# vvvwo/KSS-ICP

Hardware: AMD Instinct MI355X
Metric: icp_iterations_per_sec (higher is better)
Workload: dtype f32; 1 GPU; C2: one 100000x100000 uniform-sphere pair per GPU, 50 fixed ICP iterations + fitness pass per step (exact NN + cov reduce + host 3x3 SVD), R_z(10deg), jitter 1e-3; n_src=100000, n_tgt=100000, pairs_per_gpu=1, nn_engine=cell list + brute-force fallback, nn_arithmetic=reference (no fma)

## Files before the change

### kss-icp_amd/csrc/kss_api.hip

```cpp
#pragma clang fp contract(off)

#include "kss_ctx.hpp"

extern "C" {

int kss_version(void) { return KSS_VERSION; }

const char* kss_status_string(int s) {
    switch (s) {
        case KSS_OK: return "ok";
        case KSS_ERR_ARG: return "invalid argument";
        case KSS_ERR_HIP: return "HIP runtime error";
        case KSS_ERR_NOMEM: return "out of memory";
        case KSS_ERR_NODEVICE: return "no usable GPU device";
        case KSS_ERR_CAPACITY: return "output buffer too small";
        case KSS_ERR_RCCL: return "RCCL error";
        case KSS_ERR_DEGENERATE: return "degenerate point-to-plane system";
        default: return "unknown status";
    }
}

const char* kss_last_error(const kss_ctx* ctx) { return ctx ? ctx->err.c_str() : ""; }

static int ctx_create_common(int device_id, void* stream, bool borrow, kss_ctx** out) {
// ... 63 lines not shown

void* kss_ctx_stream(kss_ctx* c) { return c ? (void*)c->stream : nullptr; }

int kss_ctx_set_nn_mode(kss_ctx* c, int nn_mode) {
    if (!c || nn_mode < KSS_NN_AUTO || nn_mode > KSS_NN_GRID) return KSS_ERR_ARG;
    c->nn_mode = nn_mode;
    return KSS_OK;
}

int kss_profile_enable(kss_ctx* c, int on) {
    if (!c) return KSS_ERR_ARG;
    c->prof = on > 0 ? on : 0;
    for (int k = 0; k < KSS_K_COUNT; ++k) c->prof_tick[k] = 0;
    if (c->prof) {
        HIPCHK(c, hipSetDevice(c->device));
        while (c->ev_pool.size() < 4096) {
            kss_ctx::EvPair ep;
            if (hipEventCreate(&ep.a) != hipSuccess) break;
            if (hipEventCreate(&ep.b) != hipSuccess) { hipEventDestroy(ep.a); break; }
            c->ev_pool.push_back(ep);
        }
    }
    return KSS_OK;
}
int kss_grid_stats(kss_ctx* c, double out[8]) {
    if (!c || !out) return KSS_ERR_ARG;
    for (int k = 0; k < 8; ++k) out[k] = c->grid_stats[k];
    return KSS_OK;
}
int kss_debug_grid_evals(kss_ctx* c, double out[2]) {
    if (!c || !out) return KSS_ERR_ARG;
    out[0] = c->evals_sum; out[1] = c->evals_launches;
    c->evals_sum = 0.0; c->evals_launches = 0.0;
    return KSS_OK;
}

int kss_debug_grid_stamps(kss_ctx* c, unsigned long long* out, int64_t cap) {
    if (!c || !out) return KSS_ERR_ARG;
    if (c->stamps_nblk > 0 && c->g_stamps.p) {
        hipStreamSynchronize(c->stream);
        c->last_stamps.resize((size_t)c->stamps_nblk * 16);
        if (hipMemcpy(c->last_stamps.data(), (const unsigned long long*)c->g_stamps.p + (size_t)(c->stamps_seq & 1) * c->stamps_nblk * 16,
                      c->last_stamps.size() * sizeof(unsigned long long), hipMemcpyDeviceToHost) != hipSuccess) return KSS_ERR_HIP;
    }
    const int64_t n = std::min<int64_t>(cap, (int64_t)c->last_stamps.size());
    for (int64_t i = 0; i < n; ++i) out[i] = c->last_stamps[(size_t)i];
    return (int)n;
}
int kss_profile_reset(kss_ctx* c) {
    if (!c) return KSS_ERR_ARG;
    HIPCHK(c, hipStreamSynchronize(c->stream));
    prof_collect(c);
    for (int k = 0; k < KSS_K_COUNT; ++k) { c->prof_ms[k] = 0; c->prof_n[k] = 0; }
    return KSS_OK;
}
int kss_profile_event_overhead(kss_ctx* c, double* ms) {
    if (!c || !ms) return KSS_ERR_ARG;
    HIPCHK(c, hipSetDevice(c->device));
    hipEvent_t a = nullptr, b = nullptr;
    HIPCHK(c, hipEventCreate(&a));
    HIPCHK(c, hipEventCreate(&b));
    for (int i = 0; i < 16; ++i) launch_empty(c->stream);
    HIPCHK(c, hipStreamSynchronize(c->stream));
    double tot = 0.0;
    const int reps = 200;
    for (int i = 0; i < reps; ++i) {
// ... 977 lines not shown
```

### kss-icp_amd/csrc/kss_ctx.hpp

```cpp
#pragma once
#include <dlfcn.h>
#include <hip/hip_runtime.h>

#include <algorithm>
#include <atomic>
#include <chrono>
#include <cmath>
#include <cstdio>
#include <cstdlib>
#include <cstring>
#include <mutex>
#include <string>
#include <thread>
#include <vector>

#include "kss_internal.hpp"
#include "kss_host_pool.hpp"

using namespace kss;

struct DevBuf {
    void* p = nullptr;
    size_t cap = 0;
};

struct kss_ctx {
    int device = 0;
    int cu_count = 0;
    hipStream_t stream = nullptr;
    bool own_stream = false;
    std::string err;
    int nn_mode = KSS_NN_AUTO;
    double grid_stats[8] = {0, 0, 0, 0, 0, 0, 0, 0};
    double last_setup_ms = 0, last_loop_ms = 0;
    double t_launch_us = 0, t_wait_us = 0, t_host_us = 0;
    bool timing = false;
    bool tables_staged = false;
    int64_t stats_ns = -1, stats_nt = -1;

    DevBuf tgt4, src0, cur[2], keys, partials, sums, nn_work, red_work, pair_red, state, cs, scratch_a,
        scratch_b, scratch_c, stage_src, stage_tgt, stage_idx, stage_d2, stage_out, g_counts, g_start, g_cursor,
        g_bsums, g_sorted, g_list, g_count, g_bbox, g_partials, g_start2, g_pairs, g_stamps, g_pos, g_nnst, res_pos, res_wc, res_perm, pack_seg, reg_s, reg_t, reg_p, reg_all, reg_f, reg_g, oct_pts, oct_cen, oct_a, oct_b, oct_tmp, pre_partials, pre_state, g_rowpair, g_gate;
    DevBuf p2l_idx, p2l_d2, p2l_perm, p2l_rows, p2l_nrm, p2l_n64;
    DevBuf trim_rows, trim_state;
    HostPool pool;
    std::vector<kss_ctx*> workers;
    std::vector<unsigned long long> last_stamps;
    int stamps_nblk = 0; unsigned long long stamps_seq = 0;
    std::vector<float> h_bbox;
    unsigned int* h_box = nullptr; unsigned int* h_box_dev = nullptr; size_t h_box_bytes = 0;
    unsigned box_tag = 0; int box_rows = 0;
    double evals_sum = 0.0, evals_launches = 0.0;
    void* h_sums = nullptr;  size_t h_sums_cap = 0;
    void* h_sums_dev = nullptr;
    void* h_p2l = nullptr; size_t h_p2l_cap = 0;
    void* h_p2l_dev = nullptr;
    unsigned long long* h_seq = nullptr;
    unsigned long long* h_seq_dev = nullptr;
    size_t h_seq_bytes = 0;
    struct Gated {
        int supported = -1;
        bool want_next = false;
        bool pending = false;
        bool chain = false;
        int steps_left = 0;
        int max_steps = 1;
        int slot = 0;
        unsigned long long seq = 0;
        int32_t stamp = 0;
        const void* d_in = nullptr; void* d_out = nullptr;
        bool fma = false, full = false, want_full = false; double max_d2 = 0.0;
    } gated;
    bool ws_dirty = false;
    bool defer_wait = false;
    PairState* h_xf = nullptr; PairState* h_xf_dev = nullptr;
    bool fit_last = false;
    bool nn_have = false;
    PairState* bar_state = nullptr; int bar_state_cap = 0; bool bar_state_failed = false;
    unsigned int* gate_bar = nullptr;
    unsigned int* res_gate = nullptr; int res_gate_cap = 0; bool res_gate_failed = false;
    unsigned res_launches = 0;
    double res_passes = 0.0;
    int cand_cap = 0, cand_cap_pad = -1, cand_cap_fma = -1;
    int spec_judge = -1; double spec_threshold = 0.0; bool spec_ran = false, spec_cancelled = false;
    std::chrono::steady_clock::time_point res_backoff[2] = {};
    unsigned long long seq = 0;
    void* h_state = nullptr; size_t h_state_cap = 0;

    int prof = 0;
    unsigned prof_tick[KSS_K_COUNT] = {};
    struct EvPair { hipEvent_t a, b; };
    std::vector<EvPair> ev[KSS_K_COUNT];
    std::vector<EvPair> ev_pool;
    double prof_ms[KSS_K_COUNT] = {0};
    int64_t prof_n[KSS_K_COUNT] = {0};
};

// ... 126 lines not shown
```

### kss-icp_amd/csrc/kss_engine.hip

```cpp
#pragma clang fp contract(off)

#include <emmintrin.h>

#include "kss_ctx.hpp"

namespace kss {

static int restore_zero_at_rest(kss_ctx* c);
static bool resident_gate_available(kss_ctx* c, int npairs);

static int resident_rows_limit(kss_ctx* c) {
    if (c->cu_count <= 0) {
        hipDeviceProp_t prop;
        c->cu_count = hipGetDeviceProperties(&prop, c->device) == hipSuccess && prop.multiProcessorCount > 0 ? prop.multiProcessorCount : 1;
        (void)hipGetLastError();
    }
    return c->cu_count;
}

constexpr int PUB_PAIRS = 32;
static int ensure_pub(kss_ctx* c, int npairs = PUB_PAIRS);

struct PairGeom {
    int64_t ns, nt;
// ... 547 lines not shown
    }
    return c->gated.supported == 1;
}

static void gated_release(kss_ctx* c, const PairState& st, int skip) {
    if (c->gate_bar) {
        int words[16];
        std::memcpy(words, &st, sizeof st);
        words[14] = skip;
        unsigned int* slot = c->gate_bar + 32 * c->gated.slot;
        static const long torn_at = getenv("KSS_TEST_TORN_GATE") ? atol(getenv("KSS_TEST_TORN_GATE")) : -1;
        static long released = 0;
        const bool torn = ++released == torn_at;
        for (int pass = torn ? 0 : 1; pass < 2; ++pass) {
            for (int g = 0; g < 5; ++g) {
                const unsigned tag = (unsigned)c->gated.stamp + kss_mix3((unsigned)words[3 * g], (unsigned)words[3 * g + 1], (unsigned)words[3 * g + 2]);
                const int w1 = pass == 0 && g == 1 ? words[3 * g + 1] ^ 0x00010000 : words[3 * g + 1];
                const __m128i v = _mm_set_epi32((int)tag, words[3 * g + 2], w1, words[3 * g]);
                _mm_store_si128((__m128i*)(slot + 4 * g), v);
            }
            _mm_sfence();
            if (pass == 0) {
                const auto t0 = std::chrono::steady_clock::now();
                while (std::chrono::duration<double, std::micro>(std::chrono::steady_clock::now() - t0).count() < 200.0) __builtin_ia32_pause();
            }
        }
    } else {
        PairState* rec = &c->h_xf[c->gated.slot];
        for (int k = 0; k < 12; ++k) rec->m[k] = st.m[k];
        rec->active = st.active; rec->apply = st.apply; rec->pad[0] = skip;
        __atomic_store_n(&rec->pad[1], c->gated.stamp, __ATOMIC_RELEASE);
    }
    kss_ctx::Gated& G = c->gated;
    if (!skip && --G.steps_left > 0) {
        G.slot ^= 1;
        G.stamp += 1;
        G.seq += 1;
        const void* in = G.d_out; G.d_out = const_cast<void*>(G.d_in); G.d_in = in;
    } else {
        G.pending = false;
        G.steps_left = 0;
    }
}

static void gated_cancel(kss_ctx* c) {
    if (!c->gated.pending) return;
    PairState none;
    std::memset(&none, 0, sizeof none);
    gated_release(c, none, 1);
}

struct GatedGuard {
    kss_ctx* c;
    explicit GatedGuard(kss_ctx* c_) : c(c_) {}
    ~GatedGuard() { gated_cancel(c); c->gated.want_next = false; }
};

static PassArgs pass_args(kss_ctx* c, const IcpPlan& pl, const float4* d_in, float4* d_out, double max_d2,
                          int32_t* d_idx_out, float* d_d2_out) {
    PassArgs a;
    std::memset(&a, 0, sizeof a);
    a.src_in = d_in; a.src_out = d_out;
    a.cell_start = (const int32_t*)c->g_start.p + 1;
    a.sorted = (const float4*)c->g_sorted.p;
    a.tgt4 = (const float4*)c->tgt4.p;
    a.nn_win = (float4*)c->g_pos.p;
    a.nn_state = (float2*)c->g_nnst.p;
    static const float skin = getenv("KSS_SKIN") ? (float)atof(getenv("KSS_SKIN")) : 0.25f;
    a.skin = skin;
    a.chain_len = 1;
    static const int gate_polls = getenv("KSS_GATE_POLLS") ? atoi(getenv("KSS_GATE_POLLS")) : (1 << 22);
    a.gate_polls = gate_polls;
    a.chained = d_in != (const float4*)c->src0.p ? 1 : c->fit_last ? 2 : 0;
    a.src_last0 = (const float4*)c->cur[0].p; a.src_last1 = (const float4*)c->cur[1].p;
    a.keys = (unsigned long long*)c->keys.p;
    a.list = (int32_t*)c->g_list.p; a.list_count = (int32_t*)c->g_count.p;
    a.total_rows = pl.total_rows;
    static const bool noprev = getenv("KSS_GRID_NOPREV") != nullptr;
    a.use_prev = !noprev && c->nn_have ? 1 : 0;
    a.max_d2 = max_d2;
    a.rows = (Granule*)c->partials.p;
    a.pub = c->h_seq_dev;
    a.idx_out = d_idx_out; a.d2_out = d_d2_out;
    {
        static const long torn_at = getenv("KSS_TEST_TORN_SLOT") ? atol(getenv("KSS_TEST_TORN_SLOT")) : -1;
        static long launches = 0;
        a.test_torn = torn_at > 0 && ++launches == torn_at ? 1 : 0;
    }
    if (pl.gridb) {
        a.pairs = (const GridPairDev*)c->g_pairs.p;
        a.row_pair = (const int32_t*)c->g_rowpair.p;
        a.defer_pairs = pl.npairs > resident_rows_limit(c) ? pl.npairs : 0;
    } else {
        a.pair0 = pl.gpairs[0];
    }
    return a;
}

static int nn_pass(kss_ctx* c, const IcpPlan& pl, bool fma, const float4* d_in, float4* d_out, double max_d2,
            int32_t* d_idx_out, float* d_d2_out, bool full, const int* active = nullptr) {
    PairState* hs = (PairState*)c->h_state;
    if (pl.grid) {
        PassArgs a = pass_args(c, pl, d_in, d_out, max_d2, d_idx_out, d_d2_out);
        const int nblk = grid_pass_blocks(pl.total_rows);
        static const int stamps_mode = getenv("KSS_GRID_STAMPS") ? atoi(getenv("KSS_GRID_STAMPS")) : 0;
        unsigned long long* stamps2 = nullptr;
        if (stamps_mode == 1) {
            KCHK(ensure(c, c->g_stamps, (size_t)nblk * 16 * sizeof(unsigned long long)));
            HIPCHK(c, hipMemsetAsync(c->g_stamps.p, 0, (size_t)nblk * 16 * sizeof(unsigned long long), c->stream));
            a.stamps = (unsigned long long*)c->g_stamps.p;
        } else if (stamps_mode == 2) {
            KCHK(ensure(c, c->g_stamps, (size_t)nblk * 32 * sizeof(unsigned long long)));
            stamps2 = (unsigned long long*)c->g_stamps.p;
            c->stamps_nblk = nblk;
        }
        const auto tl0 = c->timing ? std::chrono::steady_clock::now() : std::chrono::steady_clock::time_point();
        unsigned long long want_seq = 0;
        bool via_gate = false;
        kss_ctx::Gated& G = c->gated;
        const bool plain_args = !a.stamps && !d_idx_out && !d_d2_out;
        if (G.pending && G.d_in == (const void*)d_in && G.d_out == (void*)d_out && G.fma == fma && G.full == full && G.max_d2 == max_d2 && plain_args) {
            want_seq = G.seq;
            c->seq = std::max(c->seq, G.seq);
            if (G.chain && c->prof > 0) c->prof_n[KSS_K_GRID_CHAIN_PASS] += 1;
            via_gate = true;
            static const long drop_at = getenv("KSS_TEST_DROP_GATE") ? atol(getenv("KSS_TEST_DROP_GATE")) : -1;
            static long releases = 0;
            if (++releases == drop_at) { G.pending = false; G.steps_left = 0; }
            else gated_release(c, hs[0], 0);
        } else {
            gated_cancel(c);
            ProfScope ps(c, KSS_K_GRID_NN);
            a.ps0 = hs[0];
            a.seq = ++c->seq;
            if (stamps2) a.stamps = stamps2 + (size_t)(a.seq & 1) * nblk * 16;
            launch_grid_pass(c->stream, fma, full, false, true, a);
            c->nn_have = true;
            want_seq = c->seq;
        }
        HIPCHK(c, hipGetLastError());
        const bool next_sampled = c->prof == 1 || (c->prof > 1 && c->prof_tick[KSS_K_GRID_NN] % (unsigned)c->prof == 0);
        static const bool want_chain = getenv("KSS_CHAIN") == nullptr || atoi(getenv("KSS_CHAIN")) != 0;
        int len = 1;
        if (G.want_next && !G.pending && plain_args && gated_available(c) && want_chain && c->gate_bar &&
            (pl.total_rows <= resident_rows_limit(c) || pl.total_rows == 1))
            len = std::max(1, std::min(G.max_steps, 1 << 16));
        if (G.want_next && !G.pending && plain_args && gated_available(c) && (len > 1 || !next_sampled)) {
            if (c->prof > 1 && len == 1) ++c->prof_tick[KSS_K_GRID_NN];
            float4* nxt_out = d_out == (float4*)c->cur[0].p ? (float4*)c->cur[1].p : (float4*)c->cur[0].p;
            G.slot ^= 1;
            G.stamp = (G.stamp + 1) & 0x7fffffff;
            if (G.stamp == 0 || G.stamp > 0x7fffffff - len - 1) G.stamp = 1;
            PassArgs n = pass_args(c, pl, d_out, nxt_out, max_d2, nullptr, nullptr);
            n.ps0 = hs[0];
            n.gate_seq = G.stamp;
            if (c->gate_bar) {
                n.state = nullptr;
                n.gate_dev = c->gate_bar;
                n.gate_slot = G.slot;
                n.chain_len = len;
                n.src_alt = d_out;
            } else {
                n.state = c->h_xf_dev + G.slot;
                n.gate_dev = (unsigned int*)c->g_gate.p;
            }
            n.seq = c->seq + 1;
            if (stamps2) n.stamps = stamps2 + (size_t)(n.seq & 1) * nblk * 16;
            if (len > 1) {
                ProfScope ps(c, KSS_K_GRID_CHAIN, true);
                launch_grid_pass(c->stream, fma, G.want_full, false, true, n);
            } else {
                launch_grid_pass(c->stream, fma, G.want_full, false, true, n);
            }
            G.chain = len > 1;
            G.pending = true; G.steps_left = len; G.seq = n.seq; G.d_in = d_out; G.d_out = nxt_out; G.fma = fma; G.full = G.want_full; G.max_d2 = max_d2;
            if (hipGetLastError() != hipSuccess) { gated_cancel(c); G.supported = 0; }
        }
        const auto tl1 = c->timing ? std::chrono::steady_clock::now() : std::chrono::steady_clock::time_point();
        {
            bool not_published = false;
            int rcw = wait_seq(c, 1, want_seq, nullptr, &not_published);
            if (rcw != KSS_OK && via_gate && not_published) {
                G.pending = false; G.steps_left = 0;
                c->err.clear();
                std::fprintf(stderr, "[kss] a waiting kernel was not answered in time and left; the pass is launched again\n");
                c->ws_dirty = true;
                KCHK(restore_zero_at_rest(c));
                ProfScope ps(c, KSS_K_GRID_NN);
                a.ps0 = hs[0];
                a.seq = ++c->seq;
                launch_grid_pass(c->stream, fma, full, false, true, a);
                HIPCHK(c, hipGetLastError());
                want_seq = c->seq;
                rcw = wait_seq(c, 1, want_seq);
            }
            KCHK(rcw);
        }
        if (stamps2) c->stamps_seq = want_seq;
        if (c->timing) {
            const auto tl2 = std::chrono::steady_clock::now();
            c->t_launch_us += std::chrono::duration<double, std::micro>(tl1 - tl0).count();
            c->t_wait_us += std::chrono::duration<double, std::micro>(tl2 - tl1).count();
        }
        if (a.stamps && !stamps2) {
            c->last_stamps.resize((size_t)nblk * 16);
            HIPCHK(c, hipMemcpy(c->last_stamps.data(), a.stamps, c->last_stamps.size() * sizeof(unsigned long long), hipMemcpyDeviceToHost));
            for (int b = 0; b < nblk; ++b) c->evals_sum += (double)c->last_stamps[(size_t)b * 16 + 10];
            c->evals_launches += 1.0;
        }
        if (((const double*)c->h_sums)[NSUMS - 1] > 0.0) {
            gated_cancel(c);
            c->gated.want_next = false;
            KCHK(stage_tables(c, pl));
            {
                PairState one;
                std::memset(&one, 0, sizeof one);
                one.active = 1;
                HIPCHK(c, hipMemcpy(c->state.p, &one, sizeof one, hipMemcpyHostToDevice));
            }
            if (getenv("KSS_LIST_CHECK")) {
                HIPCHK(c, hipStreamSynchronize(c->stream));
                int32_t cnt = -1;
                HIPCHK(c, hipMemcpy(&cnt, c->g_count.p, sizeof cnt, hipMemcpyDeviceToHost));
                const int64_t ns0 = pl.g[0].ns;
                std::vector<int32_t> l((size_t)std::max<int64_t>(0, std::min<int64_t>(cnt, ns0)));
                if (!l.empty()) HIPCHK(c, hipMemcpy(l.data(), c->g_list.p, l.size() * sizeof(int32_t), hipMemcpyDeviceToHost));
                int64_t bad = 0;
                for (int32_t v : l) bad += v < 0 || v >= ns0;
                std::fprintf(stderr, "[kss] list check: count %d of %lld sources (column 19 said %.0f), %lld entries out of range, nn table %zu items, S %d\n",
                             cnt, (long long)ns0, ((const double*)c->h_sums)[NSUMS - 1], (long long)bad, pl.nn.size(), pl.S);
                if (cnt < 0 || cnt > ns0 || bad) return set_err(c, KSS_ERR_HIP, "list check failed");
            }
            {
                ProfScope ps(c, KSS_K_NN_SWEEP);
                launch_nn_sweep_list(c->stream, pl.S, fma, (const NNWork*)c->nn_work.p, (int)pl.nn.size(), (const PairState*)c->state.p,
                                     d_out, (const float4*)c->tgt4.p, (unsigned long long*)c->keys.p, (const int32_t*)c->g_list.p,
                                     (const int32_t*)c->g_count.p);
            }
            HIPCHK(c, hipMemsetAsync(c->g_count.p, 0, sizeof(int32_t), c->stream));
            {
                ProfScope ps(c, KSS_K_CORR_REDUCE);
                PassArgs r = pass_args(c, pl, d_in, d_out, max_d2, d_idx_out, d_d2_out);
                r.ps0 = hs[0];
                r.seq = ++c->seq;
                launch_grid_pass(c->stream, fma, true, false, false, r);
            }
            HIPCHK(c, hipGetLastError());
            KCHK(wait_seq(c, 1, c->seq));
        }
        ((double*)c->h_sums)[NSUMS - 1] = 0.0;
        return KSS_OK;
    }
    if (pl.gridb) {
        PassArgs a = pass_args(c, pl, d_in, d_out, max_d2, d_idx_out, d_d2_out);
        a.state = (const PairState*)c->state.p;
        if (c->bar_state && c->bar_state_cap >= pl.npairs) {
            _mm_sfence();
            a.state = c->bar_state;
        }
        static const int host_state_rows = [] { const char* e = getenv("KSS_BATCH_HOST_STATE_ROWS"); return e ? atoi(e) : 32768; }();
        if (a.state != c->bar_state && pl.total_rows <= host_state_rows) {
            void* dev = nullptr;
            if (hipHostGetDevicePointer(&dev, c->h_state, 0) == hipSuccess && dev) a.state = (const PairState*)dev;
        }
        if (a.state == (const PairState*)c->state.p)
            HIPCHK(c, hipMemcpyAsync(c->state.p, hs, (size_t)pl.npairs * sizeof(PairState), hipMemcpyHostToDevice, c->stream));
        const int nblk = grid_pass_blocks(pl.total_rows);
        if (getenv("KSS_GRID_STAMPS")) {
            KCHK(ensure(c, c->g_stamps, (size_t)nblk * 16 * sizeof(unsigned long long)));
            HIPCHK(c, hipMemsetAsync(c->g_stamps.p, 0, (size_t)nblk * 16 * sizeof(unsigned long long), c->stream));
            a.stamps = (unsigned long long*)c->g_stamps.p;
        }
        {
            ProfScope ps(c, KSS_K_GRID_NN);
            a.seq = ++c->seq;
// ... 100 lines not shown
    cv.mse_rel = P.euclidean_fitness_epsilon;
    cv.mse_abs = P.abs_mse_epsilon;
    cv.fixed_iterations = P.fixed_iterations != 0;
    return cv;
}
static inline void trace_row(const kss_icp_params& P, const double* s, int ncol, const float* tk, double* trace_trim = nullptr,
                             const double* info = nullptr) {
    if (!P.trace_n || *P.trace_n >= P.trace_cap) return;
    if (P.trace_sums) std::memcpy(P.trace_sums + (size_t)(*P.trace_n) * ncol, s, (size_t)ncol * sizeof(double));
    if (P.trace_Tk) std::memcpy(P.trace_Tk + (size_t)(*P.trace_n) * 16, tk, 16 * sizeof(float));
    if (trace_trim) std::memcpy(trace_trim + (size_t)(*P.trace_n) * KSS_TRIM_NINFO, info, KSS_TRIM_NINFO * sizeof(double));
    ++*P.trace_n;
}
static inline void fill_result(kss_icp_result& r, const float fin[16], int iterations, int converged, int state, double last_mse,
                               double fitness, int pair) {
    std::memcpy(r.T, fin, 16 * sizeof(float));
    r.iterations = iterations; r.converged = converged; r.state = state;
    r.last_mse = last_mse; r.fitness = fitness; r.pair_id = pair;
}
static int fitness_pass(kss_ctx* c, const IcpPlan& pl, const kss_icp_params& P, const float* fin, const int* iters, const int* state,
                        bool claim_last, PairState* bar, int32_t* d_idx, float* d_d2, kss_icp_result* results) {
    const int np = pl.npairs;
    PairState* hs = (PairState*)c->h_state;
    const bool claim = claim_last && (pl.grid || pl.gridb);
    for (int p = 0; p < np; ++p) {
        set_state(hs[p], fin + (size_t)p * 16, 1, 1);
        if (claim && iters[p] >= 1 && state[p] != KSS_STATE_NO_CORRESPONDENCES && state[p] != KSS_STATE_DEGENERATE)
            hs[p].pad[0] = 1 + ((iters[p] - 1) & 1);
        mirror_state(bar, p, hs[p]);
    }
    c->fit_last = claim;
    struct FitGuard { kss_ctx* c; ~FitGuard() { c->fit_last = false; } } fit_guard{c};
    c->gated.want_next = false;
    KCHK(nn_pass(c, pl, P.nn_fma != 0, (const float4*)c->src0.p, (float4*)c->cur[0].p, P.max_corr_dist * P.max_corr_dist, d_idx, d_d2, true));
    const double* hsum = (const double*)c->h_sums;
    if (P.allreduce) {
        double v[2] = {hsum[17], (double)pl.g[0].ns};
        if (P.allreduce(P.allreduce_user, v, 2) != 0) return set_err(c, KSS_ERR_RCCL, "icp: the allreduce callback failed");
        results[0].fitness = v[0] / v[1];
    } else {
        for (int p = 0; p < np; ++p) results[p].fitness = hsum[(size_t)p * NSUMS + 17] / (double)pl.g[p].ns;
    }
    if (d_idx) {
        const size_t n0 = (size_t)pl.g[0].ns;
        if (P.fitness_idx) HIPCHK(c, hipMemcpyAsync(P.fitness_idx, d_idx, n0 * sizeof(int32_t), hipMemcpyDeviceToHost, c->stream));
        if (P.fitness_d2) HIPCHK(c, hipMemcpyAsync(P.fitness_d2, d_d2, n0 * sizeof(float), hipMemcpyDeviceToHost, c->stream));
        HIPCHK(c, hipStreamSynchronize(c->stream));
    }
    return KSS_OK;
}

static bool resident_capacities(const IcpPlan& pl, int* ntc_out, int* tabc_out) {
    int64_t max_nt = 0;
    for (int p = 0; p < pl.npairs; ++p) {
        if (pl.g[p].ns > (int64_t)RES_SMAX * RES_THREADS || pl.g[p].nt > 65534) return false;
        max_nt = std::max(max_nt, pl.g[p].nt);
    }
    const int ntc = (int)((max_nt + 3 + 63) / 64 * 64);
    const int64_t avail = ((int64_t)RES_LDS_MAX - (int64_t)resident_lds_bytes(ntc, 0)) / 2 / 8 * 8;
    if (avail < 16) return false;
    int64_t want = 16;
    for (int p = 0; p < pl.npairs; ++p) {
        const GridParams& gp = pl.gpairs[p].gp;
        const int64_t rows = (int64_t)gp.gy * gp.gz;
        int xs = 0;
        while (xs <= 8 && rows * (((gp.gx + (1 << xs) - 1) >> xs) + 1) > avail) ++xs;
// ... 471 lines not shown
        const int n = p1 - p0;
        if (n >= 64) {
            std::atomic<int> next{0};
            static const int kBlock = [] { const char* e = getenv("KSS_SOLVE_BLOCK"); const int v = e ? atoi(e) : 0; return v > 0 ? v : 64; }();
            c->pool.parallel_for(n, [&](int, int) {
                for (;;) {
                    const int pb = p0 + next.fetch_add(1) * kBlock;
                    if (pb >= p1) break;
                    solve(pb, std::min(p1, pb + kBlock));
                }
            });
        } else {
            solve(p0, p1);
        }
        if (stuck.load() > 0) {
            HIPCHK(c, hipStreamSynchronize(c->stream));
            for (int p = p0; p < p1; ++p) {
                if (!active[p] || solved[p]) continue;
                if (!collect_pair(c, p, pass_seq)) return set_err(c, KSS_ERR_HIP, "kernel finished without publishing its result");
            }
            poll = false;
            solve(p0, p1);
        }
        *n_finished = finished.load(std::memory_order_relaxed);
        return KSS_OK;
    };

    while (n_active > 0) {
        const float4* d_in = it == 0 ? (const float4*)c->src0.p : (const float4*)c->cur[(it - 1) & 1].p;
        float4* d_out = (float4*)c->cur[it & 1].p;
        c->gated.want_next = plan->grid && !P.allreduce && it + 1 < P.max_iterations;
        c->gated.want_full = full;
        c->gated.max_steps = P.max_iterations - (it + 1);
        c->defer_wait = plan->gridb;
        const auto tb0 = c->timing ? std::chrono::steady_clock::now() : std::chrono::steady_clock::time_point();
        const int rc_pass = nn_pass(c, *plan, P.nn_fma != 0, d_in, d_out, max_d2, nullptr, nullptr, full, active.data());
        const bool deferred = c->defer_wait;
        c->defer_wait = false;
        const auto tb1 = c->timing ? std::chrono::steady_clock::now() : std::chrono::steady_clock::time_point();
        KCHK(rc_pass);
        const unsigned long long pass_seq = c->seq;
        if (P.allreduce && P.allreduce(P.allreduce_user, (double*)c->h_sums, NSUMS) != 0)
            return set_err(c, KSS_ERR_RCCL, "icp: the allreduce callback failed");
        if (plan->gridb) was_active = active;
        int fin_now = 0;
        KCHK(solve_pairs(0, np, pass_seq, deferred, &fin_now));
        if (c->timing && deferred) {
            const auto tb2 = std::chrono::steady_clock::now();
            c->t_launch_us += std::chrono::duration<double, std::micro>(tb1 - tb0).count();
            c->t_wait_us += std::chrono::duration<double, std::micro>(tb2 - tb1).count();
        }
        if (plan->gridb) {
            double fallback = 0.0, act = 0.0;
            for (int p = 0; p < np; ++p)
                if (was_active[p]) { fallback += hsum[(size_t)p * NSUMS + NSUMS - 1]; act += (double)plan->g[p].ns; }
            if (fallback > 0.10 * act && !getenv("KSS_GRID_NOSWITCH")) {
                std::vector<int64_t> ns(np), nt(np);
                for (int p = 0; p < np; ++p) { ns[p] = plan->g[p].ns; nt[p] = plan->g[p].nt; }
                KCHK(build_plan(c, ns.data(), nt.data(), np, pl_in.shared_target, P.nn_sources_per_thread, P.nn_target_splits, KSS_NN_BRUTE, brute_plan));
                brute_plan.src_in_cell_order = true;
                KCHK(stage_plan(c, brute_plan));
                plan = &brute_plan;
            }
        }
        n_active -= fin_now;
        ++it;
// ... 64 lines not shown
    const auto t2 = std::chrono::steady_clock::now();
    c->last_setup_ms = std::chrono::duration<double, std::milli>(t1 - t0).count();
    c->last_loop_ms = std::chrono::duration<double, std::milli>(t2 - t1).count();
    if (c->timing)
        std::fprintf(stderr, "[kss] setup %.3f ms, loop+fitness %.3f ms (fused launches: enqueue %.1f us, wait %.1f us, rest = host math)\n",
                     c->last_setup_ms, c->last_loop_ms, c->t_launch_us, c->t_wait_us);
    return rc;
}

static int pair_loop(kss_ctx* c, const IcpPlan& pl, const kss_icp_params& P, const PairMode& M, const float* d_tgt, const float* d_nrm,
                     const int32_t* d_perm, kss_icp_result* res) {
    const int64_t ns = pl.g[0].ns, nt = pl.g[0].nt;
    const int ncol = M.plane ? P2L_NSUMS : NSUMS;
    Convergence cv = convergence_of(P);
    float fin[16], tk[16], I[16];
    mat4_identity(fin);
    mat4_identity(I);
    PairState* hs = (PairState*)c->h_state;
    set_state(hs[0], I, 1, 0);
    const double max_d2 = P.max_corr_dist * P.max_corr_dist;
    int32_t* d_idx = (int32_t*)c->p2l_idx.p;
    float* d_d2 = (float*)c->p2l_d2.p;
    double* d_rows = (double*)c->p2l_rows.p;
    const double* hp = (const double*)c->h_p2l;
    double* d_rec = (double*)c->h_p2l_dev;
    TrimState* d_state = (TrimState*)c->trim_state.p;
    const double* d_cut = M.trimmed ? &d_state[TRIM_NSTATE - 1].cut : nullptr;
    if (P.trace_n) *P.trace_n = 0;
    if (M.last_info) for (int q = 0; q < KSS_TRIM_NINFO; ++q) M.last_info[q] = 0.0;
    int it = 0, iters = 0, state = KSS_STATE_NOT_CONVERGED, converged = 0;
    double last_mse = 0.0;
    GatedGuard gated_guard(c);
    c->gated.want_next = false;
    while (P.max_iterations > 0) {
        const float4* d_in = it == 0 ? (const float4*)c->src0.p : (const float4*)c->cur[(it - 1) & 1].p;
        float4* d_out = (float4*)c->cur[it & 1].p;
        KCHK(nn_pass(c, pl, P.nn_fma != 0, d_in, d_out, max_d2, d_idx, d_d2, false));
        {
            ProfScope ps(c, KSS_K_CORR_REDUCE);
            if (M.trimmed) launch_trim_select(c->stream, d_d2, ns, max_d2, M.overlap, (unsigned*)c->trim_rows.p, d_state, d_rec + P2L_NSUMS);
            if (M.plane)
                launch_p2l_sums(c->stream, nullptr, d_out, d_perm, d_idx, d_d2, d_tgt, d_nrm, ns, nt, max_d2, d_rows, d_rec, d_cut);
            else
                launch_trim_point_sums(c->stream, d_out, d_perm, d_idx, d_d2, d_tgt, ns, nt, d_cut, d_rows, d_rec);
        }
        HIPCHK(c, hipGetLastError());
        HIPCHK(c, hipStreamSynchronize(c->stream));
        ++it;
        double s[P2L_NSUMS], info[KSS_TRIM_NINFO] = {};
        std::memcpy(s, hp, (size_t)ncol * sizeof(double));
        if (M.trimmed) {
            std::memcpy(info, hp + P2L_NSUMS, sizeof info);
            info[3] = s[0];
            if (M.last_info) std::memcpy(M.last_info, info, sizeof info);
        }
        if ((int)s[0] < P.min_correspondences) { state = KSS_STATE_NO_CORRESPONDENCES; break; }
        if (M.plane) {
            if (!rigid_from_p2l_sums(s, tk)) { state = KSS_STATE_DEGENERATE; break; }
        } else {
            rigid_from_sums(s, tk);
        }
        mat4_mul(tk, fin, fin);
        ++iters;
        const double mse = (M.plane ? s[28] : s[16]) / s[0];
        last_mse = mse;
        trace_row(P, s, ncol, tk, M.trimmed ? M.trace_trim : nullptr, info);
// ... 87 lines not shown
```

### kss-icp_amd/csrc/kss_grid.hip

```cpp
#pragma clang fp contract(off)

#include <hip/hip_runtime.h>

#include <cstring>

#include <rocprim/rocprim.hpp>

#include <cstdlib>

#include "kss_internal.hpp"
#include "kss_device.hpp"

namespace kss {

__global__ __launch_bounds__(256) void grid_count2_kernel(const float4* __restrict__ tgt, int nt, int nbt, const float4* __restrict__ src, int ns,
                                                          GridParams gp, int32_t* __restrict__ counts) {
    const bool is_src = (int)blockIdx.x >= nbt;
    const int i = ((int)blockIdx.x - (is_src ? nbt : 0)) * 256 + (int)threadIdx.x;
    if (i >= (is_src ? ns : nt)) return;
    const float4 p = is_src ? src[i] : tgt[i];
    const int cx = cell_coord(p.x, gp.ox, gp.inv_h, gp.gx), cy = cell_coord(p.y, gp.oy, gp.inv_h, gp.gy),
              cz = cell_coord(p.z, gp.oz, gp.inv_h, gp.gz);
    atomicAdd(&counts[(is_src ? gp.gx * gp.gy * gp.gz : 0) + (cz * gp.gy + cy) * gp.gx + cx], 1);
}
// ... 538 lines not shown
        ps = a.state[pi];
        if (!ps.active) return;
    }
    const GridParams& gp = pr.gp;
    const int32_t* __restrict__ cs = a.cell_start + pr.cell_base;
    const float4* __restrict__ sorted = a.sorted;
    constexpr int WQ = 256;
    __shared__ int2 rowq[9][WQ];
    __shared__ double shw[BS / 64][NSUMS];
    __shared__ int s_last;
    __shared__ int sh_ps[16];
    __shared__ int s_nwalk;
    __shared__ unsigned s_ent[7][BS];
    __shared__ unsigned short s_wl[BS];
    enum { WK_X, WK_Y, WK_Z, WK_IDX, WK_D2, WK_R, WK_POS, WK_FL = WK_POS, WK_COLS };
    static_assert(sizeof(PairState) == 64, "the gated launch reads the transform record as 16 dwords");
    double (*shf)[NSUMS] = reinterpret_cast<double (*)[NSUMS]>(&rowq[0][0]);
    static_assert(sizeof(double) * PASS_FG * NSUMS <= sizeof(int2) * 9 * WQ, "shf must fit inside rowq");

    const int local = (w - pr.row_base) * BS + (int)threadIdx.x;
    const bool valid = local < pr.src_n;
    const int i = pr.src_base + local;
    const int lane = threadIdx.x & 63, wave = threadIdx.x >> 6;
    bool have = false, fell_back = false;
    float qx = 0.f, qy = 0.f, qz = 0.f, d2 = 0.f;
    float4 win = make_float4(0.f, 0.f, 0.f, 0.f);
    float4 p = make_float4(0.f, 0.f, 0.f, 0.f), prevp = make_float4(0.f, 0.f, 0.f, __uint_as_float(~0u));
    float2 st = make_float2(0.f, 0.f);
    if (valid) {
        p = SEARCH ? a.src_in[i] : a.src_out[i];
        if (!SEARCH || a.use_prev) { prevp = a.nn_win[i]; st = a.nn_state[i]; }
    }
    for (int step = 0;; ++step) {
    const bool last_step = !CHAIN || step + 1 >= a.chain_len;
    const unsigned long long seq_k = a.seq + (unsigned long long)step;
    const int gate_k = a.gate_seq != 0 ? a.gate_seq + step : 0;
    unsigned int* const gate_ptr = a.gate_dev + 32 * ((a.gate_slot + step) & 1);
    float4* const src_out_k = (step & 1) ? a.src_alt : a.src_out;
    const bool last_known = a.chained == 2 && ps.pad[0] > 0;
    const bool chained_k = step > 0 || a.chained == 1 || last_known;
    const bool has_prev = __float_as_uint(prevp.w) != ~0u;
    if constexpr (SEARCH) {
        __syncthreads();
        if (threadIdx.x == 0) s_nwalk = 0;
        __syncthreads();
    }
    KSS_STAMP(13);
    if constexpr (!BATCH && SEARCH) {
        if (gate_k != 0) {
            typedef unsigned int u32x4 __attribute__((ext_vector_type(4)));
            if (a.state && w == 0 && threadIdx.x < 16) {
                const int* w32 = reinterpret_cast<const int*>(a.state);
                int v = 0, n = 0;
                bool ok = true;
                for (;;) {
                    v = __hip_atomic_load(w32 + threadIdx.x, __ATOMIC_RELAXED, __HIP_MEMORY_SCOPE_SYSTEM);
                    if (__shfl(v, 15, 64) == gate_k) break;
                    __builtin_amdgcn_s_sleep(1);
                    if (++n > a.gate_polls / 2) { ok = false; break; }
                }
                if (ok) {
                    const int g = threadIdx.x;
                    const int w0 = __shfl(v, min(3 * g, 15), 64), w1 = __shfl(v, min(3 * g + 1, 15), 64), w2 = __shfl(v, min(3 * g + 2, 15), 64);
                    if (g < 5) {
                        u32x4 o;
                        o.x = (unsigned)w0; o.y = (unsigned)w1; o.z = (unsigned)w2; o.w = (unsigned)gate_k + kss_mix3(o.x, o.y, o.z);
                        unsigned int* dst = gate_ptr + 4 * g;
                        asm volatile("global_store_dwordx4 %0, %1, off sc1" ::"v"(dst), "v"(o) : "memory");
                    }
                }
            }
            if (threadIdx.x < 8) {
                const unsigned int* src = gate_ptr + 4 * min((int)threadIdx.x, 4);
                u32x4 v;
                int n = 0;
                bool ok = true;
                for (;;) {
                    asm volatile("global_load_dwordx4 %0, %1, off sc0 sc1\n\ts_waitcnt vmcnt(0)" : "=&v"(v) : "v"(src) : "memory");
                    if (__builtin_amdgcn_ballot_w64(v.w - kss_mix3(v.x, v.y, v.z) == (unsigned)gate_k) == 0xffull) break;
                    __builtin_amdgcn_s_sleep(1);
                    if (++n > a.gate_polls) { ok = false; break; }
                }
                if (threadIdx.x < 5) { sh_ps[3 * threadIdx.x] = (int)v.x; sh_ps[3 * threadIdx.x + 1] = (int)v.y; sh_ps[3 * threadIdx.x + 2] = (int)v.z; }
                if (threadIdx.x == 0) { sh_ps[15] = gate_k; s_last = ok ? 1 : 0; }
            }
            __syncthreads();
            if (!s_last) return;
            int* d32 = reinterpret_cast<int*>(&ps);
#pragma unroll
            for (int k = 0; k < 16; ++k) d32[k] = sh_ps[k];
            if (ps.pad[0] != 0) return;
            __syncthreads();
            KSS_STAMP(9);
        }
    }
    unsigned long long key = ~0ull;
    float pold_x = p.x, pold_y = p.y, pold_z = p.z;
    if (SEARCH && last_known && valid) {
        const float4 pl = (ps.pad[0] == 1 ? a.src_last0 : a.src_last1)[i];
        pold_x = pl.x; pold_y = pl.y; pold_z = pl.z;
    }
    if (valid) {
        if constexpr (SEARCH) {
            if (ps.apply) {
                const float x = p.x, y = p.y, z = p.z;
                p.x = ((ps.m[0] * x + ps.m[1] * y) + ps.m[2] * z) + ps.m[3];
                p.y = ((ps.m[4] * x + ps.m[5] * y) + ps.m[6] * z) + ps.m[7];
                p.z = ((ps.m[8] * x + ps.m[9] * y) + ps.m[10] * z) + ps.m[11];
            }
            src_out_k[i] = p;
        }
        qx = p.x; qy = p.y; qz = p.z;
        const bool qok = (qx - qx) == 0.f && (qy - qy) == 0.f && (qz - qz) == 0.f;
        if constexpr (!SEARCH) {
            if (has_prev) {
                win = prevp;
                key = point_key<FMA>(win, qx, qy, qz);
            } else if (qok) {
                key = a.keys[i];
                if (key != ~0ull) win = a.tgt4[pr.tgt_base + (int)(unsigned)(key & 0xffffffffull)];
            }
            have = key != ~0ull;
        }
    }
    if constexpr (SEARCH) {
        bool walker = false;
        float acc_keep = 0.f;
        {
            const bool qok = valid && (qx - qx) == 0.f && (qy - qy) == 0.f && (qz - qz) == 0.f;
            const SkipOut so = skip_test<FMA>(qok, qx, qy, qz, pold_x, pold_y, pold_z, prevp, st, chained_k, a.skin, gp.h);
            walker = so.walker;
            key = so.key;
            acc_keep = so.acc;
// ... 28 lines not shown
        {
            const unsigned fl = s_ent[WK_FL][threadIdx.x];
            have = (fl & 1u) != 0u; fell_back = (fl & 2u) != 0u;
            win = make_float4(__uint_as_float(s_ent[WK_X][threadIdx.x]), __uint_as_float(s_ent[WK_Y][threadIdx.x]), __uint_as_float(s_ent[WK_Z][threadIdx.x]), 0.f);
            key = ((unsigned long long)s_ent[WK_D2][threadIdx.x] << 32) | (unsigned long long)s_ent[WK_IDX][threadIdx.x];
            if (CHAIN && !last_step) {
                if (walker) {
                    prevp = make_float4(win.x, win.y, win.z, __uint_as_float(have ? (unsigned)key : ~0u));
                    st = make_float2(__uint_as_float(s_ent[WK_R][threadIdx.x]), 0.f);
                } else if (have) {
                    st.y = acc_keep;
                } else {
                    prevp.w = __uint_as_float(~0u);
                    st = make_float2(0.f, 0.f);
                }
            }
        }
        if constexpr (BATCH) {
            p = make_float4(0.f, 0.f, 0.f, 0.f);
            if (valid) p = src_out_k[i];
            qx = p.x; qy = p.y; qz = p.z;
        }
    }
    if (valid && have) {
        d2 = __uint_as_float((unsigned)(key >> 32));
        const int oi = __float_as_int(p.w);
        if (a.idx_out) a.idx_out[oi] = (int)(unsigned)(key & 0xffffffffull);
        if (a.d2_out) a.d2_out[oi] = d2;
    }
    KSS_STAMP(1);

    const double d2d = have ? (double)d2 : 0.0;
    const bool kept = have && !(d2d > a.max_d2);
    wave_row<FULL>(have, kept, fell_back, qx, qy, qz, win, d2d, shw[wave]);
    __syncthreads();
    double r = 0.0;
    if (threadIdx.x < NSUMS)
#pragma unroll
        for (int ww = 0; ww < BS / 64; ++ww) r += shw[ww][threadIdx.x];
    KSS_STAMP(2);

    double v = 0.0 + r;
    if (pr.n_rows > 1) {
        Granule* const rows = a.rows + (int64_t)pr.row_base * NSUMS;
        if (threadIdx.x < NSUMS) row_put(rows + (int64_t)(w - pr.row_base) * NSUMS, threadIdx.x, r, seq_k);
        KSS_STAMP(3);
        if (w != pr.row_base || a.defer_pairs) {
            if (last_step) return;
            continue;
        }
        if (!rows_total<PASS_FG>(rows, pr.n_rows, seq_k, 1 << 20, shf, &s_last, v)) return;
    }
    if (threadIdx.x < NSUMS) {
        if (!FULL && (threadIdx.x == 17 || threadIdx.x == 18)) v = 0.0;
        const int64_t slot = (int64_t)pi * NSUMS + threadIdx.x;
        if (a.test_torn && threadIdx.x == 5) {
            pub_put(a.pub, slot, v, seq_k, 0x00100000u);
            asm volatile("s_waitcnt vmcnt(0)" ::: "memory");
            for (int k = 0; k < 400; ++k) __builtin_amdgcn_s_sleep(64);
        }
        pub_put(a.pub, slot, v, seq_k);
        KSS_STAMP(4);
    }
    if (last_step) break;
    }
#undef KSS_STAMP
}

#ifndef KSS_BATCH2_WAVES
#define KSS_BATCH2_WAVES 5
#endif
template <bool FMA, bool FULL, int WQ>
__global__ __launch_bounds__(256, KSS_BATCH2_WAVES) void gridb_pass_kernel(const PassArgs a) {
#define KSS_STAMP(k) do { if (a.stamps && threadIdx.x == 0) a.stamps[(size_t)blockIdx.x * 16 + (k)] = __builtin_amdgcn_s_memrealtime(); } while (0)
    KSS_STAMP(0);
    constexpr int BS = PASS_BS, NT = 256, SPL = BS / NT;
    static_assert(SPL == 2 && WQ <= NT, "two sources per lane");
    const int per_xcd = (int)gridDim.x / 8;
    const int w = ((int)blockIdx.x % 8) * per_xcd + (int)blockIdx.x / 8;
    if (w >= a.total_rows) return;
    const int pi = a.row_pair[w];
    const GridPairDev pr = a.pairs[pi];
    const PairState ps = a.state[pi];
    if (!ps.active) return;
    const GridParams& gp = pr.gp;
    const int32_t* __restrict__ cs = a.cell_start + pr.cell_base;
    const float4* __restrict__ sorted = a.sorted;
// ... 483 lines not shown
```

### kss-icp_amd/csrc/kss_internal.hpp

```cpp
#pragma once
#include <hip/hip_runtime.h>

#include <algorithm>
#include <cfloat>
#include <cmath>
#include <cstdint>
#include <functional>
#include <string>
#include <vector>

#include "../../include/kssicp.h"
#include "kss_host_math.hpp"

namespace kss {

struct alignas(16) PairState {
    float m[12];
    int32_t active;
    int32_t apply;
    int32_t pad[2];
};

struct alignas(16) NNWork {
    int32_t pair;
// ... 48 lines not shown
    int32_t tgt_pad;
    int32_t row_base, n_rows;
    int32_t sorted_base;
};

struct PackSeg {
    int64_t in_off;
    int64_t out_base;
    int64_t n;
};

struct alignas(16) Granule { unsigned long long bits, seq; };

struct PassArgs {
    const float4* src_in; float4* src_out;
    const int32_t* cell_start;
    const float4* sorted;
    const float4* tgt4;
    float4* nn_win;
    float2* nn_state;
    int32_t chained;
    const float4* src_last0; const float4* src_last1;
    float skin;
    unsigned long long* keys;
    int32_t* list; int32_t* list_count;
    const GridPairDev* pairs;
    const int32_t* row_pair;
    const PairState* state;
    GridPairDev pair0; PairState ps0;
    int32_t total_rows, use_prev;
    int32_t gate_polls;
    int32_t chain_len, gate_slot;
    float4* src_alt;
    int32_t gate_seq;
    int32_t defer_pairs;
    unsigned int* gate_dev;
    double max_d2;
    Granule* rows;
    unsigned long long* pub; unsigned long long seq;
    int32_t* idx_out; float* d2_out;
    unsigned long long* stamps;
    int32_t test_torn;
};

constexpr int RES_THREADS = 1024;
constexpr int RES_SMAX = 10;
constexpr int RES_NQ = 640;
constexpr int RES_QW = 4;
constexpr int RES_G = 4;
constexpr int RES_LDS_MAX = 160 * 1024 - 256;
constexpr unsigned RES_STAMP_ANY = 4095u;
__device__ __forceinline__ void res_store_exit_flag(unsigned long long* flags, int pair, unsigned tag, unsigned note = 0u) {
    typedef unsigned int u32x4 __attribute__((ext_vector_type(4)));
    u32x4 o;
    o.x = tag; o.y = (unsigned)pair; o.z = note; o.w = kss_mix3(o.x, o.y, o.z);
    unsigned long long* dst = flags + 2 * (int64_t)pair;
    asm volatile("global_store_dwordx4 %0, %1, off sc0 sc1" ::"v"(dst), "v"(o) : "memory");
}
struct ResArgs {
    const GridPairDev* pairs;
    const int32_t* cell_start;
    const float4* sorted;
    const float4* src0;
    unsigned int* gate;
    unsigned long long* pub;
    unsigned long long seq0;
// ... 181 lines not shown
```

Baseline: 81050 iterations/s.

## Extend persistent gated chain to cover first iteration and fitness pass

The persistent chained grid pass now starts at the very first ICP iteration, which was previously a standalone launch, and extends one step past the last iteration to run the fitness pass inside the same resident kernel. On the final step the kernel reads the original source points and computes full sums. This removes a separate kernel launch and host round trip at each end of the 50-iteration loop. In exchange it adds more gate/sequence bookkeeping, a new fit-step protocol (pad[0]==2), and debug launch counters.

```diff
diff --git a/kss-icp_amd/csrc/kss_api.hip b/kss-icp_amd/csrc/kss_api.hip
--- a/kss-icp_amd/csrc/kss_api.hip
+++ b/kss-icp_amd/csrc/kss_api.hip
@@ -119,6 +119,12 @@
     if (!c || !out) return KSS_ERR_ARG;
     out[0] = c->evals_sum; out[1] = c->evals_launches;
     c->evals_sum = 0.0; c->evals_launches = 0.0;
+    return KSS_OK;
+}
+
+int kss_debug_launches(kss_ctx* c, int64_t out[8]) {
+    if (!c || !out) return KSS_ERR_ARG;
+    for (int k = 0; k < 8; ++k) out[k] = c->dbg_launches[k];
     return KSS_OK;
 }
 
diff --git a/kss-icp_amd/csrc/kss_ctx.hpp b/kss-icp_amd/csrc/kss_ctx.hpp
--- a/kss-icp_amd/csrc/kss_ctx.hpp
+++ b/kss-icp_amd/csrc/kss_ctx.hpp
@@ -50,6 +50,7 @@
     std::vector<float> h_bbox;
     unsigned int* h_box = nullptr; unsigned int* h_box_dev = nullptr; size_t h_box_bytes = 0;
     unsigned box_tag = 0; int box_rows = 0;
+    int64_t dbg_launches[8] = {0, 0, 0, 0, 0, 0, 0, 0};
     double evals_sum = 0.0, evals_launches = 0.0;
     void* h_sums = nullptr;  size_t h_sums_cap = 0;
     void* h_sums_dev = nullptr;
@@ -62,7 +63,10 @@
         int supported = -1;
         bool want_next = false;
         bool pending = false;
+        bool want_fit = false;
         bool chain = false;
+        bool fit = false;
+        unsigned long long seq0 = 0;
         int steps_left = 0;
         int max_steps = 1;
         int slot = 0;
diff --git a/kss-icp_amd/csrc/kss_engine.hip b/kss-icp_amd/csrc/kss_engine.hip
--- a/kss-icp_amd/csrc/kss_engine.hip
+++ b/kss-icp_amd/csrc/kss_engine.hip
@@ -603,6 +603,8 @@
         __atomic_store_n(&rec->pad[1], c->gated.stamp, __ATOMIC_RELEASE);
     }
     kss_ctx::Gated& G = c->gated;
+    c->dbg_launches[6] += 1;
+    if (G.chain && skip != 1) c->dbg_launches[skip == 2 ? 3 : 2] += 1;
     if (!skip && --G.steps_left > 0) {
         G.slot ^= 1;
         G.stamp += 1;
@@ -624,7 +626,7 @@
 struct GatedGuard {
     kss_ctx* c;
     explicit GatedGuard(kss_ctx* c_) : c(c_) {}
-    ~GatedGuard() { gated_cancel(c); c->gated.want_next = false; }
+    ~GatedGuard() { gated_cancel(c); c->gated.want_next = false; c->gated.want_fit = false; }
 };
 
 static PassArgs pass_args(kss_ctx* c, const IcpPlan& pl, const float4* d_in, float4* d_out, double max_d2,
@@ -690,32 +692,72 @@
         bool via_gate = false;
         kss_ctx::Gated& G = c->gated;
         const bool plain_args = !a.stamps && !d_idx_out && !d_d2_out;
-        if (G.pending && G.d_in == (const void*)d_in && G.d_out == (void*)d_out && G.fma == fma && G.full == full && G.max_d2 == max_d2 && plain_args) {
+        auto answer_lost = [&]() -> bool {
+            static const long drop_at = getenv("KSS_TEST_DROP_GATE") ? atol(getenv("KSS_TEST_DROP_GATE")) : -1;
+            static long releases = 0;
+            c->dbg_launches[5] += 1;
+            return ++releases == drop_at;
+        };
+        static const bool want_chain = getenv("KSS_CHAIN") == nullptr || atoi(getenv("KSS_CHAIN")) != 0;
+        auto chain_ok = [&]() -> bool {
+            return plain_args && gated_available(c) && want_chain && c->gate_bar && (pl.total_rows <= resident_rows_limit(c) || pl.total_rows == 1);
+        };
+        static const bool want_ends = getenv("KSS_CHAIN_ENDS") == nullptr || atoi(getenv("KSS_CHAIN_ENDS")) != 0;
+        const bool fit_in = G.want_fit && want_ends && c->prof == 0;
+        const int iters_left = G.want_next ? std::max(0, std::min(G.max_steps, 1 << 16)) : 0;
+        float4* d_out_eff = d_out;
+        bool in_chain = false;
+        if (c->fit_last && d_in == (const float4*)c->src0.p && G.pending && G.fit && hs[0].pad[0] > 0 && G.fma == fma && G.max_d2 == max_d2 && plain_args) {
+            want_seq = G.seq;
+            c->seq = std::max(c->seq, G.seq);
+            via_gate = in_chain = true;
+            d_out_eff = (float4*)G.d_out;
+            if (answer_lost()) { G.pending = false; G.steps_left = 0; }
+            else gated_release(c, hs[0], 2);
+        } else if (G.pending && G.d_in == (const void*)d_in && G.d_out == (void*)d_out && G.fma == fma && G.full == full && G.max_d2 == max_d2 && plain_args) {
             want_seq = G.seq;
             c->seq = std::max(c->seq, G.seq);
             if (G.chain && c->prof > 0) c->prof_n[KSS_K_GRID_CHAIN_PASS] += 1;
             via_gate = true;
-            static const long drop_at = getenv("KSS_TEST_DROP_GATE") ? atol(getenv("KSS_TEST_DROP_GATE")) : -1;
-            static long releases = 0;
-            if (++releases == drop_at) { G.pending = false; G.steps_left = 0; }
+            in_chain = G.chain;
+            if (answer_lost()) { G.pending = false; G.steps_left = 0; }
             else gated_release(c, hs[0], 0);
+        } else if (gated_cancel(c);
+                   d_in == (const float4*)c->src0.p && !c->fit_last && want_ends && c->prof == 0 && iters_left + (fit_in ? 1 : 0) > 0 && chain_ok()) {
+            const int len = 1 + iters_left + (fit_in ? 1 : 0);
+            float4* alt = d_out == (float4*)c->cur[0].p ? (float4*)c->cur[1].p : (float4*)c->cur[0].p;
+            G.slot ^= 1;
+            G.stamp = (G.stamp + 1) & 0x7fffffff;
+            if (G.stamp == 0 || G.stamp > 0x7fffffff - len - 1) G.stamp = 1;
+            PassArgs n = a;
+            n.ps0 = hs[0];
+            n.gate_seq = G.stamp; n.state = nullptr; n.gate_dev = c->gate_bar; n.gate_slot = G.slot;
+            n.chain_len = len; n.src_alt = alt;
+            n.chain_first = 1; n.chain_fit = fit_in ? 1 : 0; n.src_fit = (const float4*)c->src0.p;
+            n.seq = ++c->seq;
+            if (stamps2) n.stamps = stamps2 + (size_t)(n.seq & 1) * nblk * 16;
+            launch_grid_pass(c->stream, fma, full, false, true, n);
+            c->dbg_launches[1] += 1; c->dbg_launches[2] += 1;
+            c->nn_have = true;
+            want_seq = n.seq;
+            in_chain = true;
+            G.chain = true; G.fit = fit_in; G.seq0 = n.seq;
+            G.pending = true; G.steps_left = len - 1; G.seq = n.seq + 1; G.d_in = d_out; G.d_out = alt; G.fma = fma; G.full = full; G.max_d2 = max_d2;
         } else {
-            gated_cancel(c);
             ProfScope ps(c, KSS_K_GRID_NN);
             a.ps0 = hs[0];
             a.seq = ++c->seq;
             if (stamps2) a.stamps = stamps2 + (size_t)(a.seq & 1) * nblk * 16;
             launch_grid_pass(c->stream, fma, full, false, true, a);
+            c->dbg_launches[0] += 1;
             c->nn_have = true;
             want_seq = c->seq;
         }
         HIPCHK(c, hipGetLastError());
         const bool next_sampled = c->prof == 1 || (c->prof > 1 && c->prof_tick[KSS_K_GRID_NN] % (unsigned)c->prof == 0);
-        static const bool want_chain = getenv("KSS_CHAIN") == nullptr || atoi(getenv("KSS_CHAIN")) != 0;
         int len = 1;
-        if (G.want_next && !G.pending && plain_args && gated_available(c) && want_chain && c->gate_bar &&
-            (pl.total_rows <= resident_rows_limit(c) || pl.total_rows == 1))
-            len = std::max(1, std::min(G.max_steps, 1 << 16));
+        if (G.want_next && !G.pending && chain_ok()) len = std::max(1, iters_left + (fit_in ? 1 : 0));
+        const bool with_fit = fit_in && len > 1;
         if (G.want_next && !G.pending && plain_args && gated_available(c) && (len > 1 || !next_sampled)) {
             if (c->prof > 1 && len == 1) ++c->prof_tick[KSS_K_GRID_NN];
             float4* nxt_out = d_out == (float4*)c->cur[0].p ? (float4*)c->cur[1].p : (float4*)c->cur[0].p;
@@ -731,6 +773,7 @@
                 n.gate_slot = G.slot;
                 n.chain_len = len;
                 n.src_alt = d_out;
+                n.chain_fit = with_fit ? 1 : 0; n.src_fit = (const float4*)c->src0.p;
             } else {
                 n.state = c->h_xf_dev + G.slot;
                 n.gate_dev = (unsigned int*)c->g_gate.p;
@@ -743,7 +786,8 @@
             } else {
                 launch_grid_pass(c->stream, fma, G.want_full, false, true, n);
             }
-            G.chain = len > 1;
+            c->dbg_launches[len > 1 ? 1 : 0] += 1;
+            G.chain = len > 1; G.fit = with_fit; G.seq0 = n.seq;
             G.pending = true; G.steps_left = len; G.seq = n.seq; G.d_in = d_out; G.d_out = nxt_out; G.fma = fma; G.full = G.want_full; G.max_d2 = max_d2;
             if (hipGetLastError() != hipSuccess) { gated_cancel(c); G.supported = 0; }
         }
@@ -761,13 +805,15 @@
                 a.ps0 = hs[0];
                 a.seq = ++c->seq;
                 launch_grid_pass(c->stream, fma, full, false, true, a);
+                c->dbg_launches[0] += 1;
                 HIPCHK(c, hipGetLastError());
                 want_seq = c->seq;
+                in_chain = false; d_out_eff = d_out;
                 rcw = wait_seq(c, 1, want_seq);
             }
             KCHK(rcw);
         }
-        if (stamps2) c->stamps_seq = want_seq;
+        if (stamps2) c->stamps_seq = in_chain ? G.seq0 : want_seq;
         if (c->timing) {
             const auto tl2 = std::chrono::steady_clock::now();
             c->t_launch_us += std::chrono::duration<double, std::micro>(tl1 - tl0).count();
@@ -782,6 +828,7 @@
         if (((const double*)c->h_sums)[NSUMS - 1] > 0.0) {
             gated_cancel(c);
             c->gated.want_next = false;
+            c->dbg_launches[4] += 1;
             KCHK(stage_tables(c, pl));
             {
                 PairState one;
@@ -805,13 +852,13 @@
             {
                 ProfScope ps(c, KSS_K_NN_SWEEP);
                 launch_nn_sweep_list(c->stream, pl.S, fma, (const NNWork*)c->nn_work.p, (int)pl.nn.size(), (const PairState*)c->state.p,
-                                     d_out, (const float4*)c->tgt4.p, (unsigned long long*)c->keys.p, (const int32_t*)c->g_list.p,
+                                     d_out_eff, (const float4*)c->tgt4.p, (unsigned long long*)c->keys.p, (const int32_t*)c->g_list.p,
                                      (const int32_t*)c->g_count.p);
             }
             HIPCHK(c, hipMemsetAsync(c->g_count.p, 0, sizeof(int32_t), c->stream));
             {
                 ProfScope ps(c, KSS_K_CORR_REDUCE);
-                PassArgs r = pass_args(c, pl, d_in, d_out, max_d2, d_idx_out, d_d2_out);
+                PassArgs r = pass_args(c, pl, d_in, d_out_eff, max_d2, d_idx_out, d_d2_out);
                 r.ps0 = hs[0];
                 r.seq = ++c->seq;
                 launch_grid_pass(c->stream, fma, true, false, false, r);
@@ -978,6 +1025,7 @@
     c->fit_last = claim;
     struct FitGuard { kss_ctx* c; ~FitGuard() { c->fit_last = false; } } fit_guard{c};
     c->gated.want_next = false;
+    c->gated.want_fit = false;
     KCHK(nn_pass(c, pl, P.nn_fma != 0, (const float4*)c->src0.p, (float4*)c->cur[0].p, P.max_corr_dist * P.max_corr_dist, d_idx, d_d2, true));
     const double* hsum = (const double*)c->h_sums;
     if (P.allreduce) {
@@ -1515,6 +1563,7 @@
         c->gated.want_next = plan->grid && !P.allreduce && it + 1 < P.max_iterations;
         c->gated.want_full = full;
         c->gated.max_steps = P.max_iterations - (it + 1);
+        c->gated.want_fit = plan->grid && !P.allreduce && P.compute_fitness && !P.fitness_idx && !P.fitness_d2;
         c->defer_wait = plan->gridb;
         const auto tb0 = c->timing ? std::chrono::steady_clock::now() : std::chrono::steady_clock::time_point();
         const int rc_pass = nn_pass(c, *plan, P.nn_fma != 0, d_in, d_out, max_d2, nullptr, nullptr, full, active.data());
@@ -1645,6 +1694,7 @@
     double last_mse = 0.0;
     GatedGuard gated_guard(c);
     c->gated.want_next = false;
+    c->gated.want_fit = false;
     while (P.max_iterations > 0) {
         const float4* d_in = it == 0 ? (const float4*)c->src0.p : (const float4*)c->cur[(it - 1) & 1].p;
         float4* d_out = (float4*)c->cur[it & 1].p;
diff --git a/kss-icp_amd/csrc/kss_grid.hip b/kss-icp_amd/csrc/kss_grid.hip
--- a/kss-icp_amd/csrc/kss_grid.hip
+++ b/kss-icp_amd/csrc/kss_grid.hip
@@ -594,10 +594,12 @@
         if (!SEARCH || a.use_prev) { prevp = a.nn_win[i]; st = a.nn_state[i]; }
     }
     for (int step = 0;; ++step) {
-    const bool last_step = !CHAIN || step + 1 >= a.chain_len;
+    bool last_step = !CHAIN || step + 1 >= a.chain_len;
+    bool fit = false;
     const unsigned long long seq_k = a.seq + (unsigned long long)step;
-    const int gate_k = a.gate_seq != 0 ? a.gate_seq + step : 0;
-    unsigned int* const gate_ptr = a.gate_dev + 32 * ((a.gate_slot + step) & 1);
+    const int gstep = CHAIN ? step - a.chain_first : step;
+    const int gate_k = a.gate_seq != 0 && gstep >= 0 ? a.gate_seq + gstep : 0;
+    unsigned int* const gate_ptr = a.gate_dev + 32 * ((a.gate_slot + gstep) & 1);
     float4* const src_out_k = (step & 1) ? a.src_alt : a.src_out;
     const bool last_known = a.chained == 2 && ps.pad[0] > 0;
     const bool chained_k = step > 0 || a.chained == 1 || last_known;
@@ -606,6 +608,14 @@
         __syncthreads();
         if (threadIdx.x == 0) s_nwalk = 0;
         __syncthreads();
+    }
+    float4 p_fit = make_float4(0.f, 0.f, 0.f, 0.f);
+    bool p_fit_in = false;
+    if constexpr (CHAIN) {
+        if (a.chain_fit && step > 0 && step + 1 >= a.chain_len) {
+            if (valid) p_fit = a.src_fit[i];
+            p_fit_in = true;
+        }
     }
     KSS_STAMP(13);
     if constexpr (!BATCH && SEARCH) {
@@ -651,7 +661,8 @@
             int* d32 = reinterpret_cast<int*>(&ps);
 #pragma unroll
             for (int k = 0; k < 16; ++k) d32[k] = sh_ps[k];
-            if (ps.pad[0] != 0) return;
+            if (CHAIN && a.chain_fit && ps.pad[0] == 2) { fit = true; last_step = true; }
+            else if (ps.pad[0] != 0) return;
             __syncthreads();
             KSS_STAMP(9);
         }
@@ -661,6 +672,12 @@
     if (SEARCH && last_known && valid) {
         const float4 pl = (ps.pad[0] == 1 ? a.src_last0 : a.src_last1)[i];
         pold_x = pl.x; pold_y = pl.y; pold_z = pl.z;
+    }
+    if constexpr (CHAIN) {
+        if (fit) {
+            if (!p_fit_in && valid) p_fit = a.src_fit[i];
+            p = p_fit;
+        }
     }
     if (valid) {
         if constexpr (SEARCH) {
@@ -755,7 +772,8 @@
 
     const double d2d = have ? (double)d2 : 0.0;
     const bool kept = have && !(d2d > a.max_d2);
-    wave_row<FULL>(have, kept, fell_back, qx, qy, qz, win, d2d, shw[wave]);
+    if (CHAIN && !FULL && fit) wave_row<true>(have, kept, fell_back, qx, qy, qz, win, d2d, shw[wave]);
+    else wave_row<FULL>(have, kept, fell_back, qx, qy, qz, win, d2d, shw[wave]);
     __syncthreads();
     double r = 0.0;
     if (threadIdx.x < NSUMS)
@@ -775,7 +793,7 @@
         if (!rows_total<PASS_FG>(rows, pr.n_rows, seq_k, 1 << 20, shf, &s_last, v)) return;
     }
     if (threadIdx.x < NSUMS) {
-        if (!FULL && (threadIdx.x == 17 || threadIdx.x == 18)) v = 0.0;
+        if (!FULL && !fit && (threadIdx.x == 17 || threadIdx.x == 18)) v = 0.0;
         const int64_t slot = (int64_t)pi * NSUMS + threadIdx.x;
         if (a.test_torn && threadIdx.x == 5) {
             pub_put(a.pub, slot, v, seq_k, 0x00100000u);
diff --git a/kss-icp_amd/csrc/kss_internal.hpp b/kss-icp_amd/csrc/kss_internal.hpp
--- a/kss-icp_amd/csrc/kss_internal.hpp
+++ b/kss-icp_amd/csrc/kss_internal.hpp
@@ -104,6 +104,9 @@
     int32_t gate_polls;
     int32_t chain_len, gate_slot;
     float4* src_alt;
+    int32_t chain_first;
+    int32_t chain_fit;
+    const float4* src_fit;
     int32_t gate_seq;
     int32_t defer_pairs;
     unsigned int* gate_dev;
```

After: 78340 iterations/s. 0.967x the previous value.
